# cvigilv/SimSpread.jl

Measured on AMD Instinct MI355X. Metric: predicted edges/sec + achieved HBM GB/s, W*R SpMM, higher is better.
Workload: dtype f32

## Files before the change

### simspread.jl_amd/csrc/assemble.hip

```cpp
#include <cstdlib>
#include <cstring>
#include <hip/hip_runtime.h>
#include <rocprim/rocprim.hpp>

#include "graph.hpp"

namespace ss {

static inline int grid_for(int64_t work, int block, int cap = 256 * 16) {
  int64_t g = ceil_div(work, block);
  if (g < 1) g = 1;
  if (g > cap) g = cap;
  return (int)g;
}

__global__ void scan_tail_kernel(const int* in, int* out, int64_t n) { out[n] = out[n - 1] + in[n - 1]; }

static int exclusive_scan_int(const int* in, int* out, int64_t n) {
  hipStream_t st = ctx().stream;
  if (n == 0) {
    SS_HIP(hipMemsetAsync(out, 0, sizeof(int), st));
    return SS_OK;
  }
  size_t bytes = 0;
// ... 973 lines not shown
    }
  }
}

template <class T>
int csell_build(const DevCsr<T>& in, int KC, int QT, DevCsell<T>& out) {
  hipStream_t st = ctx().stream;
  if (KC < 1 || KC > 32767) return fail(SS_EINVAL, "compact sliced ELL: chunk size out of range");
  const int rowb = QT * (int)sizeof(T);
  if (rowb != 16 && rowb != 32 && rowb != 64 && rowb != 128 && rowb != 256)
    return fail(SS_EINVAL, "compact sliced ELL: tile rows must be 16, 32, 64, 128 or 256 bytes");
  out.ok = false;
  out.rows = in.rows; out.cols = in.cols; out.nnz = in.nnz; out.binary = in.binary;
  out.KC = KC; out.QT = QT;
  out.nchunks = (int)(in.cols > 0 ? ceil_div(in.cols, KC) : 1);
  out.nslices = (int)ceil_div(in.rows, 64);
  const int64_t nblocks = (int64_t)out.nchunks * out.nslices;
  if (nblocks <= 0 || nblocks >= (1LL << 24)) return SS_OK;
  DevBuf<int> steps, pairs, base;
  SS_TRY(out.np.alloc((size_t)(nblocks + 1) * 64));
  SS_TRY(steps.alloc(nblocks + 1));
  SS_TRY(pairs.alloc(nblocks + 1));
  SS_TRY(base.alloc(nblocks + 2));
  SS_HIP(hipMemsetAsync(out.np.p + (size_t)nblocks * 64, 0, 64 * sizeof(unsigned short), st));
  const unsigned grid = (unsigned)(nblocks < (1 << 20) ? nblocks : (1 << 20));
  hipLaunchKernelGGL(csell_count_kernel, dim3(grid), dim3(64), 0, st, in.ptr.p, in.idx.p, in.rows, KC, out.nslices,
                     nblocks, out.np.p, steps.p, pairs.p);
  SS_LAUNCH_CHECK();
  SS_TRY(exclusive_scan_int(pairs.p, base.p, nblocks));
  int total = 0;
  SS_TRY(read_int(base.p + nblocks, &total));
  if (total < 0) return SS_OK;
  out.npairs = total;
  SS_TRY(out.desc.alloc((size_t)(nblocks + 1) * 2));
  hipLaunchKernelGGL(csell_desc_kernel, dim3(grid_for(nblocks + 1, 256)), dim3(256), 0, st, base.p, steps.p, nblocks, out.desc.p);
  SS_LAUNCH_CHECK();
  SS_TRY(out.pidx.alloc((size_t)total + 64));
  SS_HIP(hipMemsetAsync(out.pidx.p + total, 0, 64 * sizeof(unsigned), st));
  if (!in.binary) {
    SS_TRY(out.pval.alloc(2 * ((size_t)total + 64)));
    SS_HIP(hipMemsetAsync(out.pval.p + 2 * (size_t)total, 0, 128 * sizeof(T), st));
  } else {
    out.pval.release();
  }
  DevBuf<int> perm;
  if (rowb < 256) SS_TRY(perm.alloc(in.nnz));
  unsigned short* p16 = reinterpret_cast<unsigned short*>(out.pidx.p);
  T* pv = in.binary ? (T*)nullptr : out.pval.p;
  if (rowb == 16)
    hipLaunchKernelGGL((csell_fill_kernel<T, 16>), dim3(grid), dim3(64), 0, st, in.ptr.p, in.idx.p, in.val.p, in.rows, KC,
                       out.nslices, nblocks, out.desc.p, perm.p, p16, pv);
  else if (rowb == 32)
    hipLaunchKernelGGL((csell_fill_kernel<T, 32>), dim3(grid), dim3(64), 0, st, in.ptr.p, in.idx.p, in.val.p, in.rows, KC,
                       out.nslices, nblocks, out.desc.p, perm.p, p16, pv);
  else if (rowb == 64)
    hipLaunchKernelGGL((csell_fill_kernel<T, 64>), dim3(grid), dim3(64), 0, st, in.ptr.p, in.idx.p, in.val.p, in.rows, KC,
                       out.nslices, nblocks, out.desc.p, perm.p, p16, pv);
  else if (rowb == 128)
    hipLaunchKernelGGL((csell_fill_kernel<T, 128>), dim3(grid), dim3(64), 0, st, in.ptr.p, in.idx.p, in.val.p, in.rows, KC,
                       out.nslices, nblocks, out.desc.p, perm.p, p16, pv);
  else
    hipLaunchKernelGGL((csell_fill_kernel<T, 256>), dim3(grid), dim3(64), 0, st, in.ptr.p, in.idx.p, in.val.p, in.rows, KC,
                       out.nslices, nblocks, out.desc.p, perm.p, p16, pv);
  SS_LAUNCH_CHECK();
  SS_HIP(hipStreamSynchronize(st));
  out.ok = true;
  return SS_OK;
}
template int csell_build<float>(const DevCsr<float>&, int, int, DevCsell<float>&);
template int csell_build<double>(const DevCsr<double>&, int, int, DevCsell<double>&);

template <class T>
__global__ void abs_range_kernel(const T* __restrict__ v, int64_t n, int* __restrict__ mm) {
  int mx = 0, mn = 0x7f7fffff;
  for (int64_t i = (int64_t)blockIdx.x * blockDim.x + threadIdx.x; i < n; i += (int64_t)gridDim.x * blockDim.x) {
    const float a = fabsf((float)v[i]);
    const int b = __float_as_int(a);
    if (a > 0.f) { mx = b > mx ? b : mx; mn = b < mn ? b : mn; }
  }
  atomicMax(&mm[0], mx);
  atomicMin(&mm[1], mn);
}

__global__ void chunk_count_kernel(const int* __restrict__ ptr, const int* __restrict__ idx, int64_t rows, int SC,
                                   int nchunks, int align, int* __restrict__ cnt, unsigned short* __restrict__ len16,
                                   int* __restrict__ toolong) {
  const int64_t total = rows * nchunks;
  for (int64_t i = (int64_t)blockIdx.x * blockDim.x + threadIdx.x; i < total; i += (int64_t)gridDim.x * blockDim.x) {
    const int c = (int)(i / rows);
    const int64_t r = i - (int64_t)c * rows;
    const int lo = ptr[r], hi = ptr[r + 1];
    const int64_t k0 = (int64_t)c * SC, k1 = k0 + SC;
    int a = lo, b = hi;
    while (a < b) { const int m = (a + b) >> 1; if (idx[m] < k0) a = m + 1; else b = m; }
    const int first = a;
    b = hi;
    while (a < b) { const int m = (a + b) >> 1; if (idx[m] < k1) a = m + 1; else b = m; }
    cnt[i] = (a - first + align - 1) / align;
    if (len16) {
      len16[i] = (unsigned short)(a - first);
      if (a - first > 65535) *toolong = 1;
    }
  }
}

constexpr int CHUNK_SCHED_ITERS = 4;
template <class T>
__global__ void chunk_fill_kernel(const int* __restrict__ ptr, const int* __restrict__ idx, const T* __restrict__ val,
                                  int64_t rows, int SC, int nchunks, int align, int sched,
                                  const int* __restrict__ off, unsigned short* __restrict__ oidx, T* __restrict__ oval) {
  const int lane = threadIdx.x & 63;
  const int64_t wave0 = ((int64_t)blockIdx.x * blockDim.x + threadIdx.x) >> 6;
  const int64_t nwaves = ((int64_t)gridDim.x * blockDim.x) >> 6;
  const int64_t total = rows * nchunks;
  for (int64_t i = wave0; i < total; i += nwaves) {
    const int c = (int)(i / rows);
    const int64_t r = i - (int64_t)c * rows;
    const int64_t o = (int64_t)off[i] * align;
    const int npad = (off[i + 1] - off[i]) * align;
    if (npad == 0) continue;
    const int lo = ptr[r], hi = ptr[r + 1];
    const int64_t k0 = (int64_t)c * SC, k1 = k0 + SC;
    int a = lo, b = hi;
    while (a < b) { const int m = (a + b) >> 1; if (idx[m] < k0) a = m + 1; else b = m; }
    const int first = a;
    b = hi;
    while (a < b) { const int m = (a + b) >> 1; if (idx[m] < k1) a = m + 1; else b = m; }
    const int n = a - first;
    if (sched && n > 32 && n <= 64 * CHUNK_SCHED_ITERS) {
      const int G = (n + 31) >> 5;
      const int L = n - 32 * (G - 1);
      int cnt = 0;
      int bank[CHUNK_SCHED_ITERS], col[CHUNK_SCHED_ITERS];
#pragma unroll
      for (int j = 0; j < CHUNK_SCHED_ITERS; ++j) {
        const int x = lane + 64 * j;
        col[j] = x < n ? (int)(idx[first + x] - k0) : -1;
        bank[j] = x < n ? (col[j] & 31) : -1;
      }
      for (int b = 0; b < 32; ++b) {
        int c = 0;
#pragma unroll
        for (int j = 0; j < CHUNK_SCHED_ITERS; ++j) c += __popcll(__ballot(bank[j] == b));
        if (lane == b) cnt = c;
      }
      int base = 0;
      for (int b = 0; b < 31; ++b) {
        const int c = __builtin_amdgcn_readlane(cnt, b);
        if (lane > b) base += c;
      }
      int run = 0;
#pragma unroll
      for (int j = 0; j < CHUNK_SCHED_ITERS; ++j) {
        int p = -1;
        for (int b = 0; b < 32; ++b) {
          const unsigned long long m = __ballot(bank[j] == b);
          const int bb = __builtin_amdgcn_readlane(base, b) + __builtin_amdgcn_readlane(run, b);
          if (bank[j] == b) p = bb + __popcll(m & ((1ull << lane) - 1ull));
          if (lane == b) run += __popcll(m);
        }
        if (p >= 0) {
          int grp, slot;
          if (p < L * G) { grp = p % G; slot = p / G; }
          else { const int q = p - L * G; grp = q % (G - 1); slot = L + q / (G - 1); }
          const int pos = grp * 32 + slot;
          oidx[o + pos] = (unsigned short)col[j];
          oval[o + pos] = val[first + lane + 64 * j];
        }
      }
      for (int x = n + lane; x < npad; x += 64) {
        oidx[o + x] = (unsigned short)SC;
        oval[o + x] = T(0);
      }
      continue;
    }
    for (int x = lane; x < npad; x += 64) {
      oidx[o + x] = x < n ? (unsigned short)(idx[first + x] - k0) : (unsigned short)SC;
      oval[o + x] = x < n ? val[first + x] : T(0);
    }
  }
}

template <class T>
int chunked_build(const DevCsr<T>& in, int SC, int align, DevChunked<T>& out) {
  hipStream_t st = ctx().stream;
  if (SC < 1 || SC > 65535) return fail(SS_EINVAL, "chunk size out of range");
  if (align != 1 && align != 4 && align != 32) return fail(SS_EINVAL, "chunk alignment must be 1, 4 or 32");
  out.rows = in.rows;
  out.cols = in.cols;
  out.nnz = in.nnz;
  out.SC = SC;
  out.align = align;
  out.binary = in.binary;
  out.nchunks = (int)(in.cols > 0 ? ceil_div(in.cols, SC) : 1);
  const int64_t total = in.rows * out.nchunks;
  SS_TRY(out.off.alloc(total + 1));
  if (total == 0) {
    SS_HIP(hipMemsetAsync(out.off.p, 0, sizeof(int), st));
    SS_TRY(out.idx.alloc(64));
    SS_TRY(out.val.alloc(64));
    SS_HIP(hipMemsetAsync(out.idx.p, 0, 64 * sizeof(unsigned short), st));
    SS_HIP(hipMemsetAsync(out.val.p, 0, 64 * sizeof(T), st));
    return SS_OK;
  }
  DevBuf<int> cnt;
  SS_TRY(cnt.alloc(total));
  DevBuf<int> toolong;
  if (align == 32) {
    SS_TRY(out.len.alloc(total));
    SS_TRY(toolong.alloc(1));
    SS_HIP(hipMemsetAsync(toolong.p, 0, sizeof(int), st));
  }
  hipLaunchKernelGGL(chunk_count_kernel, dim3(grid_for(total, 256)), dim3(256), 0, st, in.ptr.p, in.idx.p, in.rows, SC,
                     out.nchunks, align, cnt.p, align == 32 ? out.len.p : (unsigned short*)nullptr,
                     align == 32 ? toolong.p : (int*)nullptr);
  SS_LAUNCH_CHECK();
  if (align == 32) {
    int tl = 0;
    SS_TRY(read_int(toolong.p, &tl));
    out.len_ok = (tl == 0);
  }
  {
    DevBuf<int> mm;
    SS_TRY(mm.alloc(2));
    const int init[2] = {0, 0x7f7fffff};
    SS_HIP(hipMemcpyAsync(mm.p, init, sizeof(init), hipMemcpyHostToDevice, st));
    if (in.nnz > 0) {
      hipLaunchKernelGGL(abs_range_kernel<T>, dim3(grid_for(in.nnz, 256)), dim3(256), 0, st, in.val.p, in.nnz, mm.p);
      SS_LAUNCH_CHECK();
    }
    int got[2];
    SS_HIP(hipMemcpyAsync(got, mm.p, sizeof(got), hipMemcpyDeviceToHost, st));
    SS_HIP(hipStreamSynchronize(st));
    memcpy(&out.vmax, &got[0], 4);
    memcpy(&out.vmin, &got[1], 4);
    if (in.nnz == 0) out.vmax = out.vmin = 0.f;
  }
  SS_TRY(exclusive_scan_int(cnt.p, out.off.p, total));
  int units = 0;
  SS_TRY(read_int(out.off.p + total, &units));
  if (units < 0 || (int64_t)units * align >= (1LL << 31) - 64) return fail(SS_EUNSUPPORTED, "chunked operand too large");
  out.stored = (int64_t)units * align;
  SS_TRY(out.idx.alloc(out.stored + 256));
  SS_TRY(out.val.alloc(out.stored + 256));
  SS_HIP(hipMemsetAsync(out.idx.p + out.stored, 0, 256 * sizeof(unsigned short), st));
  SS_HIP(hipMemsetAsync(out.val.p + out.stored, 0, 256 * sizeof(T), st));
  const int sched = ((align == 1 || align == 32) && !env_off("SS_CHUNK_SCHED")) ? 1 : 0;
  hipLaunchKernelGGL(chunk_fill_kernel<T>, dim3(grid_for(total * 64, 256)), dim3(256), 0, st, in.ptr.p, in.idx.p,
                     in.val.p, in.rows, SC, out.nchunks, align, sched, out.off.p, out.idx.p, out.val.p);
  SS_LAUNCH_CHECK();
  SS_HIP(hipStreamSynchronize(st));
  return SS_OK;
}

template <class T>
__global__ void degree_kernel(const int* __restrict__ pa, const int* __restrict__ pb, int64_t n, int* __restrict__ k,
                              T* __restrict__ inv) {
  for (int64_t i = (int64_t)blockIdx.x * blockDim.x + threadIdx.x; i < n; i += (int64_t)gridDim.x * blockDim.x) {
    int d = pa[i + 1] - pa[i];
    if (pb) d += pb[i + 1] - pb[i];
    k[i] = d;
    inv[i] = d > 0 ? T(1) / T(d) : T(0);
  }
}

template <class T>
int graph_finalize(Graph<T>& g) {
  SS_TRY(csr_transpose(g.Xs, g.XsT));
  SS_TRY(csr_transpose(g.Ys, g.YsT));
  return graph_degrees(g);
}

template <class T>
int graph_degrees(Graph<T>& g) {
  hipStream_t st = ctx().stream;
  g.coef_drop();
  SS_TRY(g.kf.alloc(g.nf));
  SS_TRY(g.ks.alloc(g.ns));
  SS_TRY(g.kt.alloc(g.nt));
  SS_TRY(g.inv_kf.alloc(g.nf));
  SS_TRY(g.inv_ks.alloc(g.ns));
  SS_TRY(g.inv_kt.alloc(g.nt));
  if (g.nf > 0) {
    hipLaunchKernelGGL(degree_kernel<T>, dim3(grid_for(g.nf, 256)), dim3(256), 0, st, g.XsT.ptr.p, (const int*)nullptr,
                       g.nf, g.kf.p, g.inv_kf.p);
    SS_LAUNCH_CHECK();
  }
  if (g.ns > 0) {
    hipLaunchKernelGGL(degree_kernel<T>, dim3(grid_for(g.ns, 256)), dim3(256), 0, st, g.Xs.ptr.p, g.Ys.ptr.p, g.ns,
                       g.ks.p, g.inv_ks.p);
    SS_LAUNCH_CHECK();
  }
  if (g.nt > 0) {
    hipLaunchKernelGGL(degree_kernel<T>, dim3(grid_for(g.nt, 256)), dim3(256), 0, st, g.YsT.ptr.p, (const int*)nullptr,
                       g.nt, g.kt.p, g.inv_kt.p);
    SS_LAUNCH_CHECK();
  }
  SS_HIP(hipStreamSynchronize(st));
  return SS_OK;
}

template <class T>
int graph_finalize_general(Graph<T>& g) {
  hipStream_t st = ctx().stream;
  const int64_t n = g.ns;
  g.coef_drop();
  SS_TRY(g.kf.alloc(n));
  SS_TRY(g.inv_kf.alloc(n));
  SS_TRY(g.ks.alloc(n));
  SS_TRY(g.inv_ks.alloc(n));
  SS_TRY(g.kt.alloc(g.nt));
  SS_TRY(g.inv_kt.alloc(g.nt));
  if (n > 0) {
    hipLaunchKernelGGL(degree_kernel<T>, dim3(grid_for(n, 256)), dim3(256), 0, st, g.XsT.ptr.p, (const int*)nullptr, n,
                       g.kf.p, g.inv_kf.p);
    SS_LAUNCH_CHECK();
    hipLaunchKernelGGL(degree_kernel<T>, dim3(grid_for(n, 256)), dim3(256), 0, st, g.XsT.ptr.p, (const int*)nullptr, n,
                       g.ks.p, g.inv_ks.p);
    SS_LAUNCH_CHECK();
  }
  if (g.nt > 0) {
    hipLaunchKernelGGL(degree_kernel<T>, dim3(grid_for(g.nt, 256)), dim3(256), 0, st, g.YsT.ptr.p, (const int*)nullptr,
                       g.nt, g.kt.p, g.inv_kt.p);
    SS_LAUNCH_CHECK();
  }
  SS_HIP(hipStreamSynchronize(st));
  return SS_OK;
}

template <class T>
int graph_finalize_general_targets(Graph<T>& g) {
  hipStream_t st = ctx().stream;
// ... 27 lines not shown
```

### simspread.jl_amd/csrc/transfer.hip

```cpp
#include <type_traits>

#include "graph.hpp"

namespace ss {

template <class T>
struct ChunkedView {
  const int* off;
  const unsigned short* idx;
  const T* val;
  int64_t rows;
};
template <class T>
static inline ChunkedView<T> view(const DevChunked<T>& m) {
  return ChunkedView<T>{m.off.p, m.idx.p, m.val.p, m.rows};
}

template <class T>
struct TransferArgs {
  int nterms;
  CsrView<T> L[2];
  const T* inv1[2];
  const T* coef[2];
  ChunkedView<T> M[2];
// ... 78 lines not shown
  unsigned b[U];
  T cf[U];
  unsigned short j[U];
  T v[U];
};

template <int U, bool BINM>
__device__ __forceinline__ void subrows_load_buf(SubRows<float, U>& s, int first, int b_l, int n_l, float cf_l,
                                                 __amdgpu_buffer_rsrc_t ridx, __amdgpu_buffer_rsrc_t rval, int lane) {
#pragma unroll
  for (int u = 0; u < U; ++u) {
    const int src = first + u;
    s.b[u] = (unsigned)__builtin_amdgcn_readlane(b_l, src);
    s.n[u] = __builtin_amdgcn_readlane(n_l, src);
    s.cf[u] = BitsOf<float>::bcast(cf_l, src);
    s.j[u] = __builtin_amdgcn_raw_buffer_load_b16(ridx, lane * 2, (int)(s.b[u] * 2u), 0);
    s.v[u] = BINM ? 1.f : __builtin_bit_cast(float, __builtin_amdgcn_raw_buffer_load_b32(rval, lane * 4, (int)(s.b[u] * 4u), 0));
    __builtin_amdgcn_sched_barrier(0);
  }
}

template <class T, int U, bool BINM>
__device__ __forceinline__ void subrows_load(SubRows<T, U>& s, int first, int b_l, int n_l, T cf_l,
                                             const unsigned short* __restrict__ midx, const T* __restrict__ mval,
                                             int lane) {
#pragma unroll
  for (int u = 0; u < U; ++u) {
    const int src = first + u;
    s.b[u] = (unsigned)__builtin_amdgcn_readlane(b_l, src);
    s.n[u] = __builtin_amdgcn_readlane(n_l, src);
    s.cf[u] = BitsOf<T>::bcast(cf_l, src);
    const unsigned short* pi = midx + s.b[u];
    const T* pv = mval + s.b[u];
    s.j[u] = pi[lane];
    s.v[u] = BINM ? T(1) : pv[lane];
    __builtin_amdgcn_sched_barrier(0);
  }
}

template <class T, int U, bool DUAL>
__device__ __forceinline__ void subrows_fold(const SubRows<T, U>& s, T* __restrict__ acc, int astride, int dummy, int lane) {
  if constexpr (DUAL) {
    T* __restrict__ acc1 = acc + astride;
#pragma unroll
    for (int u = 0; u < U; u += 2) {
      const int ja = lane < s.n[u] ? (int)s.j[u] : dummy;
      const int jb = lane < s.n[u + 1] ? (int)s.j[u + 1] : dummy;
      const T ra = acc[ja], rb = acc1[jb];
      acc[ja] = fma(s.cf[u], s.v[u], ra);
      acc1[jb] = fma(s.cf[u + 1], s.v[u + 1], rb);
    }
  } else {
#pragma unroll
    for (int u = 0; u < U; ++u) {
      const int j = lane < s.n[u] ? (int)s.j[u] : dummy;
      acc[j] = fma(s.cf[u], s.v[u], acc[j]);
    }
  }
}

__device__ __forceinline__ int cvt_rpi(float x) {
  int r;
  asm("v_cvt_rpi_i32_f32 %0, %1" : "=v"(r) : "v"(x));
  return r;
}
template <int U>
__device__ __forceinline__ void subrows_fold_fixed(const SubRows<float, U>& s, unsigned* __restrict__ acc, int lane) {
#pragma unroll
  for (int u = 0; u < U; ++u) {
    const float v = lane < s.n[u] ? s.v[u] : 0.f;
    atomicAdd(&acc[s.j[u]], (unsigned)cvt_rpi(s.cf[u] * v));
  }
}

template <class T, int U, bool DUAL, bool FIX>
__device__ __forceinline__ void subrows_fold_any(const SubRows<T, U>& s, T* acc, int astride, int dummy, int lane) {
  if constexpr (FIX) subrows_fold_fixed<U>(s, reinterpret_cast<unsigned*>(acc), lane);
  else subrows_fold<T, U, DUAL>(s, acc, astride, dummy, lane);
}

template <class T, int AHEAD>
struct Tails {
  static constexpr int TAIL_AHEAD = AHEAD;
  int nt;
  int cb, cn;
  T ccf;
  unsigned short tj[TAIL_AHEAD];
  T tv[TAIL_AHEAD];
};

template <class T, int TAIL_AHEAD, class LD>
__device__ __forceinline__ void tails_fetch(Tails<T, TAIL_AHEAD>& t, int r0, int lane, LD&& ld) {
#pragma unroll
  for (int i = 0; i < TAIL_AHEAD; ++i) {
    if (4 * (r0 + i) >= t.nt) break;
    const unsigned b = (unsigned)__builtin_amdgcn_ds_bpermute((4 * (r0 + i) + (lane >> 4)) * 4, t.cb);
    ld(b + 64u + (unsigned)(lane & 15), t.tj[i], t.tv[i]);
    __builtin_amdgcn_sched_barrier(0);
  }
}

template <class T, int TAIL_AHEAD, class LD>
__device__ __forceinline__ void tails_begin(Tails<T, TAIL_AHEAD>& t, int b_l, int n_l, T cf_l, int lane, LD&& ld) {
  const unsigned long long longs = __ballot(n_l > 64);
  t.nt = __builtin_popcountll(longs);
  if (t.nt == 0) return;
  const int k = (int)__builtin_amdgcn_mbcnt_hi((unsigned)(longs >> 32), __builtin_amdgcn_mbcnt_lo((unsigned)longs, 0u));
  const int to4 = (n_l > 64 ? k : t.nt + lane - k) * 4;
  t.cb = __builtin_amdgcn_ds_permute(to4, b_l);
  t.cn = __builtin_amdgcn_ds_permute(to4, n_l);
  t.ccf = BitsOf<T>::push(to4, cf_l);
  tails_fetch(t, 0, lane, ld);
}

template <class T, bool BINM, bool FIX, int TAIL_AHEAD, class LD>
__device__ __forceinline__ void tails_finish(Tails<T, TAIL_AHEAD>& t, int b_l, int n_l, T cf_l, T* __restrict__ acc, int dummy,
                                             const unsigned short* __restrict__ midx, const T* __restrict__ mval, int lane,
                                             LD&& ld) {
  if (t.nt == 0) return;
  for (int r0 = 0; 4 * r0 < t.nt; r0 += TAIL_AHEAD) {
    if (r0 > 0) tails_fetch(t, r0, lane, ld);
#pragma unroll
    for (int i = 0; i < TAIL_AHEAD; ++i) {
      if (4 * (r0 + i) >= t.nt) break;
      const int from4 = (4 * (r0 + i) + (lane >> 4)) * 4;
      const int tn = __builtin_amdgcn_ds_bpermute(from4, t.cn) - 64;
      const T tcf = BitsOf<T>::pull(from4, t.ccf);
      const bool live = (lane & 15) < tn;
      if constexpr (FIX) {
        atomicAdd(reinterpret_cast<unsigned*>(acc) + (live ? (int)t.tj[i] : dummy),
                  (unsigned)cvt_rpi(live ? (float)(tcf * t.tv[i]) : 0.f));
      } else {
#pragma unroll
        for (int g = 0; g < 4; ++g) {
          const int j = (live && (lane >> 4) == g) ? (int)t.tj[i] : dummy;
          acc[j] = fma(tcf, t.tv[i], acc[j]);
        }
      }
    }
  }
  unsigned long long m = __ballot(n_l > 80);
  while (m != 0ull) {
    const int src = __builtin_ctzll(m);
    m &= m - 1ull;
    const int n = __builtin_amdgcn_readlane(n_l, src);
    const unsigned b = (unsigned)__builtin_amdgcn_readlane(b_l, src);
    const T cf = BitsOf<T>::bcast(cf_l, src);
    for (int x = 80 + lane; x < n; x += 64) {
      const int j = midx[b + x];
      const T v = BINM ? T(1) : mval[b + x];
      if constexpr (FIX) atomicAdd(reinterpret_cast<unsigned*>(acc) + j, (unsigned)cvt_rpi((float)(cf * v)));
      else acc[j] = fma(cf, v, acc[j]);
    }
  }
}

struct FixedScale {
  float scale, unscale;
};
template <class F>
__device__ __forceinline__ FixedScale fixed_scale(int lb, int le, int lane, float xmax, F&& abs_coef) {
  float sabs = 0.f;
  for (int q = lb + lane; q < le; q += 64) sabs += abs_coef(q);
#pragma unroll
  for (int o = 32; o > 0; o >>= 1) sabs += __shfl_xor(sabs, o);
  int e = 0;
  (void)frexpf(sabs * xmax, &e);
  if (!(sabs * xmax > 0.f)) e = 0;
  e = e < -90 ? -90 : (e > 120 ? 120 : e);
  return FixedScale{ldexpf(1.f, 30 - e), ldexpf(1.f, e - 30)};
}

template <class T, bool LOO, int U, bool BINM, bool DUAL, bool FIX = false, bool BUF = false, bool COEF = false>
__global__ void __launch_bounds__(TRANSFER_THREADS) transfer_kernel(TransferArgs<T> p) {
  static_assert(64 % (2 * U) == 0, "U must divide 32");
  static_assert(!COEF || (!DUAL && !FIX && !BUF), "coefficient tables serve the default family only");
  extern __shared__ __align__(16) unsigned char smem_raw[];
  T* acc = reinterpret_cast<T*>(smem_raw);
  const int astride = p.SC + 64;
  constexpr int NCOPY = DUAL ? 2 : 1;
  unsigned* bits = reinterpret_cast<unsigned*>(acc + NCOPY * astride);
  const int lane = threadIdx.x;
  int c;
  int64_t r;
  if (p.nchunks > 8 && p.nchunks % 8 == 0 && !chunks_in_turn(p)) {
    const int64_t nrows = (int64_t)gridDim.x / p.nchunks, per = nrows * 8;
    const int64_t grp = blockIdx.x / per, rem = blockIdx.x - grp * per;
    r = rem >> 3;
    c = (int)(grp * 8 + (rem & 7));
  } else {
    c = blockIdx.x % p.nchunks;
    r = blockIdx.x / p.nchunks;
  }
  const int64_t gr = p.row_ids ? (int64_t)p.row_ids[p.row_begin + r] : p.row_begin + r;
  const int64_t j0 = (int64_t)c * p.SC;
  const int jn = (int)((p.nj - j0 < p.SC) ? (p.nj - j0) : p.SC);
  const int dummy = p.SC + lane;

  for (int j = lane; j < NCOPY * astride; j += 64) acc[j] = T(0);
  if (LOO)
    for (int j = lane; j < (p.SC + 31) / 32; j += 64) bits[j] = 0u;
  __syncthreads();

  float fix_unscale = 1.f;
  for (int t = 0; t < p.nterms; ++t) {
    const CsrView<T> L = p.L[t];
    const ChunkedView<T> M = p.M[t];
    const int* __restrict__ off = M.off + (int64_t)c * M.rows;
    const unsigned short* __restrict__ midx = M.idx;
    const T* __restrict__ mval = M.val;
    const int lb = L.ptr[gr], le = L.ptr[gr + 1];
    float scale = 1.f;
    if constexpr (FIX) {
      float sabs = 0.f;
      for (int q = lb + lane; q < le; q += 64) sabs += fabsf((float)(L.val[q] * p.inv1[t][L.idx[q]]));
#pragma unroll
      for (int o = 32; o > 0; o >>= 1) sabs += __shfl_xor(sabs, o);
      int e = 0;
      (void)frexpf(sabs * p.xmax, &e);
      if (!(sabs * p.xmax > 0.f)) e = 0;
      e = e < -90 ? -90 : (e > 120 ? 120 : e);
      scale = ldexpf(1.f, 30 - e);
      fix_unscale = ldexpf(1.f, e - 30);
    }
    for (int g0 = lb; g0 < le; g0 += 64) {
      const int q = g0 + lane;
      int b_l = 0, n_l = 0;
      T cf_l = T(0);
      if constexpr (COEF) {
        if (q < le) {
          const int a = L.idx[q];
          cf_l = p.coef[t][q];
          const int o0 = off[a], o1 = off[a + 1];
          b_l = o0;
          n_l = cf_l != T(0) ? o1 - o0 : 0;
        }
      } else if (q < le) {
        const int a = L.idx[q];
        const T lv = L.val[q];
        if (LOO) {
          const int d = p.kf[a] - 1;
          cf_l = (a != (int)gr && d > 0) ? lv * (T(1) / T(d)) : T(0);
        } else {
          cf_l = lv * p.inv1[t][a];
          if constexpr (FIX) cf_l = (T)((float)cf_l * scale);
        }
        if (cf_l != T(0)) { b_l = off[a]; n_l = off[a + 1] - b_l; }
      }
      const int cnt = __builtin_amdgcn_readfirstlane((le - g0 < 64) ? (le - g0) : 64);
      SubRows<T, U> A, B;
      auto load = [&](SubRows<T, U>& sr, int first) __attribute__((always_inline)) {
        if constexpr (BUF) {
          const __amdgpu_buffer_rsrc_t ridx = __builtin_amdgcn_make_buffer_rsrc((void*)midx, 0, -1, 0x00020000);
          const __amdgpu_buffer_rsrc_t rval = __builtin_amdgcn_make_buffer_rsrc((void*)mval, 0, -1, 0x00020000);
          subrows_load_buf<U, BINM>(sr, first, b_l, n_l, cf_l, ridx, rval, lane);
        } else {
          subrows_load<T, U, BINM>(sr, first, b_l, n_l, cf_l, midx, mval, lane);
        }
      };
      auto tail_ld = [&](unsigned e, unsigned short& j, T& v) __attribute__((always_inline)) {
        if constexpr (BUF) {
          const __amdgpu_buffer_rsrc_t ridx = __builtin_amdgcn_make_buffer_rsrc((void*)midx, 0, -1, 0x00020000);
          const __amdgpu_buffer_rsrc_t rval = __builtin_amdgcn_make_buffer_rsrc((void*)mval, 0, -1, 0x00020000);
          j = __builtin_amdgcn_raw_buffer_load_b16(ridx, (int)(e * 2u), 0, 0);
          v = BINM ? 1.f : __builtin_bit_cast(float, __builtin_amdgcn_raw_buffer_load_b32(rval, (int)(e * 4u), 0, 0));
        } else {
          j = midx[e];
          v = BINM ? T(1) : mval[e];
        }
      };
      Tails<T, (BINM ? 4 : 2)> tails;
      tails_begin(tails, b_l, n_l, cf_l, lane, tail_ld);
      load(A, 0);
      for (int u0 = 0; u0 < cnt; u0 += 2 * U) {
        if (u0 + U < cnt) load(B, u0 + U);
        subrows_fold_any<T, U, DUAL, FIX>(A, acc, astride, dummy, lane);
        if (u0 + U < cnt) {
          if (u0 + 2 * U < cnt) load(A, u0 + 2 * U);
          subrows_fold_any<T, U, DUAL, FIX>(B, acc, astride, dummy, lane);
        }
      }
      tails_finish<T, BINM, FIX>(tails, b_l, n_l, cf_l, acc, dummy, midx, mval, lane, tail_ld);
    }
  }
  if (LOO) {
    const ChunkedView<T> M = p.M[0];
    const int* off = M.off + (int64_t)c * M.rows;
    for (int x = off[gr] + lane; x < off[gr + 1]; x += 64) {
      const int j = M.idx[x];
      atomicOr(&bits[j >> 5], 1u << (j & 31));
    }
  }
  __syncthreads();

  T* orow = p.out + r * p.ld + j0;
  for (int j = lane; j < jn; j += 64) {
    T z;
    T sum = DUAL ? acc[j] + acc[astride + j] : acc[j];
    if constexpr (FIX) sum = (T)((float)reinterpret_cast<const int*>(acc)[j] * fix_unscale);
    if (LOO) {
      const int d = p.ks[j0 + j] - (int)((bits[j >> 5] >> (j & 31)) & 1u);
      z = (d > 0 && (j0 + j) != gr) ? sum * (T(1) / T(d)) : T(0);
    } else {
      z = sum * p.inv2[j0 + j];
      if (p.accumulate) z += orow[j];
    }
    orow[j] = z;
  }
}

constexpr int TRANSFER_U = 8;

static bool transfer_dual() { return env_int("SS_TRANSFER_DUAL", 0) != 0; }

static int transfer_u() {
  const int u = (int)env_int("SS_TRANSFER_U", TRANSFER_U);
  return (u == 4 || u == 16) ? u : 8;
}

template <class T>
__global__ void transfer_coef_kernel(const int* __restrict__ ptr, const int* __restrict__ idx, const T* __restrict__ val,
                                     const T* __restrict__ inv1, int64_t row_begin, int64_t nrows, T* __restrict__ coef) {
  const int lo = ptr[row_begin], hi = ptr[row_begin + nrows];
  for (int64_t e = (int64_t)lo + (int64_t)blockIdx.x * blockDim.x + threadIdx.x; e < hi; e += (int64_t)gridDim.x * blockDim.x)
    coef[e] = val[e] * inv1[idx[e]];
}

enum { TB_PLAIN, TB_QFLAT, TB_WIDE, TB_WIDE2 };
constexpr int WIDE_META = 64 * 12;
constexpr int WIDE_LIST = 64;
constexpr int W2_TBL = 64 * 12;
template <int KIND, class T>
struct BlockLayout {
  static constexpr bool EXACT = KIND != TB_PLAIN;
  static constexpr int shared_bytes = KIND == TB_WIDE ? 64 : 0;
  __host__ __device__ static int64_t offs_bytes(int64_t mrows) { return (((mrows + 1) * 4 + 15) / 16) * 16; }
  __host__ __device__ static int64_t lens_bytes(int64_t mrows) { return EXACT ? ((mrows * 2 + 15) / 16) * 16 : 0; }
  __host__ __device__ static int acc_elems(int SC) { return SC + 64; }
  __host__ __device__ static int acc_bytes(int SC) {
    return KIND == TB_WIDE || KIND == TB_WIDE2 ? (((SC + 4) * 4 + 15) / 16) * 16 : acc_elems(SC) * (int)sizeof(T);
  }
  __host__ __device__ static int per_wave(int SC) {
    return acc_bytes(SC) + (KIND == TB_WIDE ? WIDE_META + WIDE_LIST : KIND == TB_WIDE2 ? 2 * W2_TBL + 4 * 64 : 0);
  }
  __device__ static unsigned char* wave_base(unsigned char* smem, int offs_b, int lens_b, int wave, int SC) {
    return smem + offs_b + lens_b + shared_bytes + (size_t)wave * (size_t)per_wave(SC);
  }
};

struct BlockWave {
  int lane, c, jn, lb, le;
  int64_t r, gr, j0;
};

template <bool EXACT, class T, class A>
__device__ __forceinline__ bool block_prologue(BlockWave& w, const TransferArgs<T>& p, int64_t nrows, int wave, int* offs,
                                               unsigned short* lens, const unsigned short* glen, A* acc, int nacc) {
  const int nw = blockDim.x >> 6;
  w.lane = threadIdx.x & 63;
  w.c = blockIdx.x % p.nchunks;
  w.r = (int64_t)(blockIdx.x / p.nchunks) * nw + wave;
  const ChunkedView<T> M = p.M[0];
  {
    const int* __restrict__ off = M.off + (int64_t)w.c * M.rows;
    for (int64_t i = threadIdx.x; i <= M.rows; i += blockDim.x) offs[i] = off[i];
    if constexpr (EXACT) {
      const unsigned short* __restrict__ gl = glen + (int64_t)w.c * M.rows;
      for (int64_t i = threadIdx.x; i < M.rows; i += blockDim.x) lens[i] = gl[i];
    }
  }
  for (int j = w.lane; j < nacc; j += 64) acc[j] = A(0);
  __syncthreads();
  return w.r < nrows;
}
template <class T>
__device__ __forceinline__ void block_row(BlockWave& w, const TransferArgs<T>& p) {
  w.gr = p.row_begin + w.r;
  w.j0 = (int64_t)w.c * p.SC;
  w.jn = (int)((p.nj - w.j0 < p.SC) ? (p.nj - w.j0) : p.SC);
  const int* lptr = p.L[0].ptr;
  w.lb = __builtin_amdgcn_readfirstlane(lptr[w.gr]);
  w.le = __builtin_amdgcn_readfirstlane(lptr[w.gr + 1]);
}

template <class T>
__device__ __forceinline__ void fixed_store(const TransferArgs<T>& p, int64_t r, int64_t j0, int jn, int lane, const void* acc,
                                            float unscale) {
  T* orow = p.out + r * p.ld + j0;
  const int* iacc = reinterpret_cast<const int*>(acc);
  for (int j = lane; j < jn; j += 64) orow[j] = (T)((float)iacc[j] * unscale) * p.inv2[j0 + j];
}

typedef float f4 __attribute__((ext_vector_type(4)));
typedef unsigned u2 __attribute__((ext_vector_type(2)));

template <bool BINM>
__device__ __forceinline__ void quad_fetch(const u2* midx4, const f4* mval4, int quad, float cfv, int rem, u2& oj, f4& ov,
                                           float& ocf) {
  ocf = cfv;
  oj = midx4[quad];
  if constexpr (BINM) ov = f4{rem > 0 ? 1.f : 0.f, rem > 1 ? 1.f : 0.f, rem > 2 ? 1.f : 0.f, rem > 3 ? 1.f : 0.f};
  else ov = mval4[quad];
}
__device__ __forceinline__ void quad_fold(unsigned* acc, u2 j, f4 v, float cf) {
  atomicAdd(acc + (j.x & 0xffffu), (unsigned)cvt_rpi(cf * v.x));
  atomicAdd(acc + (j.x >> 16), (unsigned)cvt_rpi(cf * v.y));
  atomicAdd(acc + (j.y & 0xffffu), (unsigned)cvt_rpi(cf * v.z));
  atomicAdd(acc + (j.y >> 16), (unsigned)cvt_rpi(cf * v.w));
}

__device__ __forceinline__ void raw_load(const int* lidx, const float* coef, int lb, int le, int lane, int g, int& a, float& cf) {
  const int q = lb + g * 64 + lane;
  a = 0;
  cf = 0.f;
  if (q < le) { a = lidx[q]; cf = coef[q]; }
}

template <class T, int U, bool BINM, bool FIX>
__global__ void __launch_bounds__(1024) transfer_block_kernel(TransferArgs<T> p, const T* __restrict__ coef, int64_t nrows,
                                                              int align, int offs_bytes, float xmax) {
  using Lay = BlockLayout<TB_PLAIN, T>;
  extern __shared__ __align__(16) unsigned char smem_raw[];
  int* offs = reinterpret_cast<int*>(smem_raw);
  const int wave = threadIdx.x >> 6;
  const int astride = p.SC + 64;
  T* acc = reinterpret_cast<T*>(smem_raw + offs_bytes) + (size_t)wave * Lay::acc_elems(p.SC);
  BlockWave w;
  if (!block_prologue<false>(w, p, nrows, wave, offs, nullptr, nullptr, acc, astride)) return;
  w.gr = p.row_begin + w.r;
  w.j0 = (int64_t)w.c * p.SC;
  w.jn = (int)((p.nj - w.j0 < p.SC) ? (p.nj - w.j0) : p.SC);
  const int lane = w.lane, lb = p.L[0].ptr[w.gr], le = p.L[0].ptr[w.gr + 1];
  const int dummy = p.SC + lane;
  const CsrView<T> L = p.L[0];
  const unsigned short* __restrict__ midx = p.M[0].idx;
  const T* __restrict__ mval = p.M[0].val;
  float scale = 1.f, unscale = 1.f;
  if constexpr (FIX) {
    const FixedScale fs = fixed_scale(lb, le, lane, xmax, [&](int q) __attribute__((always_inline)) { return fabsf((float)coef[q]); });
    scale = fs.scale;
    unscale = fs.unscale;
  }
  for (int g0 = lb; g0 < le; g0 += 64) {
    const int q = g0 + lane;
    int b_l = 0, n_l = 0;
    T cf_l = T(0);
    if (q < le) {
      const int a = L.idx[q];
      cf_l = coef[q];
      if constexpr (FIX) cf_l = (T)((float)cf_l * scale);
      if (cf_l != T(0)) {
        const int o0 = offs[a], o1 = offs[a + 1];
        b_l = o0 * align;
        n_l = (o1 - o0) * align;
      }
    }
    const int cnt = __builtin_amdgcn_readfirstlane((le - g0 < 64) ? (le - g0) : 64);
    SubRows<T, U> A, B;
    auto load = [&](SubRows<T, U>& sr, int first) __attribute__((always_inline)) {
      subrows_load<T, U, BINM>(sr, first, b_l, n_l, cf_l, midx, mval, lane);
    };
    auto tail_ld = [&](unsigned e, unsigned short& j, T& v) __attribute__((always_inline)) {
      j = midx[e];
      v = BINM ? T(1) : mval[e];
    };
    Tails<T, (BINM ? 4 : 2)> tails;
    tails_begin(tails, b_l, n_l, cf_l, lane, tail_ld);
    load(A, 0);
    for (int u0 = 0; u0 < cnt; u0 += 2 * U) {
      if (u0 + U < cnt) load(B, u0 + U);
      subrows_fold_any<T, U, false, FIX>(A, acc, astride, dummy, lane);
      if (u0 + U < cnt) {
        if (u0 + 2 * U < cnt) load(A, u0 + 2 * U);
        subrows_fold_any<T, U, false, FIX>(B, acc, astride, dummy, lane);
      }
    }
    tails_finish<T, BINM, FIX>(tails, b_l, n_l, cf_l, acc, dummy, midx, mval, lane, tail_ld);
  }
  if constexpr (FIX) {
    fixed_store(p, w.r, w.j0, w.jn, lane, acc, unscale);
  } else {
    T* orow = p.out + w.r * p.ld + w.j0;
    for (int j = lane; j < w.jn; j += 64) orow[j] = acc[j] * p.inv2[w.j0 + j];
  }
}

template <class T, int D, bool BINM>
__global__ void __launch_bounds__(1024) transfer_qflat_kernel(TransferArgs<T> p, const T* __restrict__ coef, int64_t nrows,
                                                             int align, int offs_bytes, int lens_bytes, float xmax,
                                                             const unsigned short* __restrict__ glen) {
  static_assert(std::is_same<T, float>::value, "fixed-point sums: fp32 graphs only");
  extern __shared__ __align__(16) unsigned char smem_raw[];
  int* offs = reinterpret_cast<int*>(smem_raw);
  unsigned short* lens = reinterpret_cast<unsigned short*>(smem_raw + offs_bytes);
  const int lane = threadIdx.x & 63;
  const int wave = __builtin_amdgcn_readfirstlane(threadIdx.x >> 6);
  const int astride = p.SC + 64;
  unsigned* acc = reinterpret_cast<unsigned*>(BlockLayout<TB_QFLAT, T>::wave_base(smem_raw, offs_bytes, lens_bytes, wave, p.SC));
  BlockWave w;
  if (!block_prologue<true>(w, p, nrows, wave, offs, lens, glen, acc, astride)) return;
  block_row(w, p);
  const ChunkedView<T> M = p.M[0];
  const CsrView<T> L = p.L[0];
  const int64_t r = w.r, j0 = w.j0;
  const int jn = w.jn, lb = w.lb, le = w.le;
  const unsigned short* __restrict__ midx = M.idx;
  const T* __restrict__ mval = M.val;
  float scale, unscale;
  {
    float sabs = 0.f;
    for (int q = lb + lane; q < le; q += 64) sabs += fabsf(coef[q]);
#pragma unroll
    for (int o = 32; o > 0; o >>= 1) sabs += __shfl_xor(sabs, o);
    int e = 0;
    (void)frexpf(sabs * xmax, &e);
    if (!(sabs * xmax > 0.f)) e = 0;
    e = e < -90 ? -90 : (e > 120 ? 120 : e);
    scale = ldexpf(1.f, 30 - e);
    unscale = ldexpf(1.f, e - 30);
  }
  const int ngroups = (le - lb + 63) >> 6;
  auto raw_load = [&](int g, int& a, float& cf) __attribute__((always_inline)) {
    const int q = lb + g * 64 + lane;
    a = 0;
    cf = 0.f;
    if (q < le) { a = L.idx[q]; cf = coef[q]; }
  };
  auto meta = [&](int a, float cf, int& b_l, int& n_l, float& cf_l) __attribute__((always_inline)) {
    cf_l = cf * scale;
    b_l = 0;
    n_l = 0;
    if (cf_l != 0.f) {
      b_l = (offs[a] * align) >> 2;
      n_l = ((int)lens[a] + 3) >> 2;
    }
  };
  int Pc = 0, dc = 0, ra, bn, nn;
  float cc = 0.f, cn, rc;
  int total = 0, nst = 0, t = 0, gcur = -1;
  raw_load(0, ra, rc); meta(ra, rc, bn, nn, cn);
  raw_load(1, ra, rc);
  bool done = false;
  auto switch_group = [&]() __attribute__((always_inline)) {
    ++gcur;
    int incl = nn;
#pragma unroll
    for (int o = 1; o < 64; o <<= 1) {
      const int up = __shfl_up(incl, o);
      if (lane >= o) incl += up;
    }
// ... 559 lines not shown
```

Measured before the change: 52.90 billion.

## Class-partition chunk tails so tail atomics avoid bank conflicts across quarter-waves

Chunk assembly now reorders long chunk rows so that the 16-entry tail after the first 64 entries holds columns whose low two bits match the row's class (row mod 4). The SpMM tail processing then groups long rows by class into quarter-wave slots, so each 16-lane group updates accumulator entries in a distinct LDS bank class. This lets the four-way serialized per-group update collapse into a single update. It also rewrites the bank-scheduling fill for up to 64 entries and adds padding and overflow paths, at the cost of a more complex build and extra padding storage.

```diff
diff --git a/simspread.jl_amd/csrc/assemble.hip b/simspread.jl_amd/csrc/assemble.hip
--- a/simspread.jl_amd/csrc/assemble.hip
+++ b/simspread.jl_amd/csrc/assemble.hip
@@ -1079,9 +1079,20 @@
   atomicMin(&mm[1], mn);
 }
 
+struct ChunkTail {
+  int real;
+  int len;
+  int stored;
+};
+__device__ __forceinline__ ChunkTail chunk_tail(int n, int m) {
+  const int t = n - 64 < 16 ? n - 64 : 16;
+  if (m >= t) return ChunkTail{t, t, n};
+  return ChunkTail{m, 16, n + 16 - m};
+}
+
 __global__ void chunk_count_kernel(const int* __restrict__ ptr, const int* __restrict__ idx, int64_t rows, int SC,
-                                   int nchunks, int align, int* __restrict__ cnt, unsigned short* __restrict__ len16,
-                                   int* __restrict__ toolong) {
+                                   int nchunks, int align, int cls_tails, int* __restrict__ cnt,
+                                   unsigned short* __restrict__ len16, int* __restrict__ toolong) {
   const int64_t total = rows * nchunks;
   for (int64_t i = (int64_t)blockIdx.x * blockDim.x + threadIdx.x; i < total; i += (int64_t)gridDim.x * blockDim.x) {
     const int c = (int)(i / rows);
@@ -1093,23 +1104,47 @@
     const int first = a;
     b = hi;
     while (a < b) { const int m = (a + b) >> 1; if (idx[m] < k1) a = m + 1; else b = m; }
-    cnt[i] = (a - first + align - 1) / align;
+    int n = a - first;
+    if (cls_tails && n > 64) {
+      const int cls = (int)(r & 3);
+      int m = 0;
+      for (int x = first; x < a; ++x) m += (int)(((idx[x] - k0) & 3) == cls);
+      n = chunk_tail(n, m).stored;
+    }
+    cnt[i] = (n + align - 1) / align;
     if (len16) {
-      len16[i] = (unsigned short)(a - first);
-      if (a - first > 65535) *toolong = 1;
-    }
-  }
-}
-
-constexpr int CHUNK_SCHED_ITERS = 4;
-template <class T>
-__global__ void chunk_fill_kernel(const int* __restrict__ ptr, const int* __restrict__ idx, const T* __restrict__ val,
-                                  int64_t rows, int SC, int nchunks, int align, int sched,
-                                  const int* __restrict__ off, unsigned short* __restrict__ oidx, T* __restrict__ oval) {
+      len16[i] = (unsigned short)n;
+      if (n > 65535) *toolong = 1;
+    }
+  }
+}
+
+__device__ __forceinline__ int chunk_sched_pos(int n, int col, int lane) {
+  const int bank = col < 0 ? -1 : (col & 31);
+  int p = 0, base = 0;
+  for (int b = 0; b < 32; ++b) {
+    const unsigned long long m = __ballot(bank == b);
+    if (bank == b) p = base + __popcll(m & ((1ull << lane) - 1ull));
+    base += __popcll(m);
+  }
+  const int L = n - 32;
+  return p < 2 * L ? (p & 1) * 32 + (p >> 1) : L + (p - 2 * L);
+}
+
+template <class T>
+__global__ void __launch_bounds__(256) chunk_fill_kernel(const int* __restrict__ ptr, const int* __restrict__ idx,
+                                                         const T* __restrict__ val, int64_t rows, int SC, int nchunks,
+                                                         int align, int sched, int cls_tails,
+                                                         const int* __restrict__ off, unsigned short* __restrict__ oidx,
+                                                         T* __restrict__ oval) {
+  __shared__ int hcol[4][64];
+  __shared__ T hval[4][64];
   const int lane = threadIdx.x & 63;
+  const int wv = (threadIdx.x >> 6) & 3;
   const int64_t wave0 = ((int64_t)blockIdx.x * blockDim.x + threadIdx.x) >> 6;
   const int64_t nwaves = ((int64_t)gridDim.x * blockDim.x) >> 6;
   const int64_t total = rows * nchunks;
+  const unsigned long long below = (1ull << lane) - 1ull;
   for (int64_t i = wave0; i < total; i += nwaves) {
     const int c = (int)(i / rows);
     const int64_t r = i - (int64_t)c * rows;
@@ -1124,46 +1159,63 @@
     b = hi;
     while (a < b) { const int m = (a + b) >> 1; if (idx[m] < k1) a = m + 1; else b = m; }
     const int n = a - first;
-    if (sched && n > 32 && n <= 64 * CHUNK_SCHED_ITERS) {
-      const int G = (n + 31) >> 5;
-      const int L = n - 32 * (G - 1);
-      int cnt = 0;
-      int bank[CHUNK_SCHED_ITERS], col[CHUNK_SCHED_ITERS];
-#pragma unroll
-      for (int j = 0; j < CHUNK_SCHED_ITERS; ++j) {
-        const int x = lane + 64 * j;
-        col[j] = x < n ? (int)(idx[first + x] - k0) : -1;
-        bank[j] = x < n ? (col[j] & 31) : -1;
+    if (cls_tails && n > 64) {
+      const int cls = (int)(r & 3);
+      int m = 0;
+      for (int x0 = 0; x0 < n; x0 += 64) {
+        const int x = x0 + lane;
+        m += __popcll(__ballot(x < n && ((idx[first + x] - k0) & 3) == cls));
       }
-      for (int b = 0; b < 32; ++b) {
-        int c = 0;
-#pragma unroll
-        for (int j = 0; j < CHUNK_SCHED_ITERS; ++j) c += __popcll(__ballot(bank[j] == b));
-        if (lane == b) cnt = c;
+      const ChunkTail tl = chunk_tail(n, m);
+      int seen_c = 0, seen_o = 0;
+      for (int x0 = 0; x0 < n; x0 += 64) {
+        const int x = x0 + lane;
+        const bool valid = x < n;
+        const int col = valid ? (int)(idx[first + x] - k0) : 0;
+        const T v = valid ? val[first + x] : T(0);
+        const unsigned long long mc = __ballot(valid && (col & 3) == cls);
+        const int rc = seen_c + __popcll(mc & below);
+        const bool in_tail = valid && (col & 3) == cls && rc < tl.real;
+        const unsigned long long mo = __ballot(valid && !in_tail);
+        const int ro = seen_o + __popcll(mo & below);
+        if (in_tail) {
+          oidx[o + 64 + rc] = (unsigned short)col;
+          oval[o + 64 + rc] = v;
+        } else if (valid) {
+          if (ro < 64) {
+            hcol[wv][ro] = col;
+            hval[wv][ro] = v;
+          } else {
+            oidx[o + 16 + ro] = (unsigned short)col;
+            oval[o + 16 + ro] = v;
+          }
+        }
+        seen_c += __popcll(mc);
+        seen_o += __popcll(mo);
       }
-      int base = 0;
-      for (int b = 0; b < 31; ++b) {
-        const int c = __builtin_amdgcn_readlane(cnt, b);
-        if (lane > b) base += c;
+      for (int x = tl.real + lane; x < tl.len; x += 64) {
+        oidx[o + 64 + x] = (unsigned short)SC;
+        oval[o + 64 + x] = T(0);
       }
-      int run = 0;
-#pragma unroll
-      for (int j = 0; j < CHUNK_SCHED_ITERS; ++j) {
-        int p = -1;
-        for (int b = 0; b < 32; ++b) {
-          const unsigned long long m = __ballot(bank[j] == b);
-          const int bb = __builtin_amdgcn_readlane(base, b) + __builtin_amdgcn_readlane(run, b);
-          if (bank[j] == b) p = bb + __popcll(m & ((1ull << lane) - 1ull));
-          if (lane == b) run += __popcll(m);
-        }
-        if (p >= 0) {
-          int grp, slot;
-          if (p < L * G) { grp = p % G; slot = p / G; }
-          else { const int q = p - L * G; grp = q % (G - 1); slot = L + q / (G - 1); }
-          const int pos = grp * 32 + slot;
-          oidx[o + pos] = (unsigned short)col[j];
-          oval[o + pos] = val[first + lane + 64 * j];
-        }
+      __builtin_amdgcn_wave_barrier();
+      const int hc = hcol[wv][lane];
+      const T hv = hval[wv][lane];
+      __builtin_amdgcn_wave_barrier();
+      const int pos = sched ? chunk_sched_pos(64, hc, lane) : lane;
+      oidx[o + pos] = (unsigned short)hc;
+      oval[o + pos] = hv;
+      for (int x = tl.stored + lane; x < npad; x += 64) {
+        oidx[o + x] = (unsigned short)SC;
+        oval[o + x] = T(0);
+      }
+      continue;
+    }
+    if (sched && n > 32 && n <= 64) {
+      const int col = lane < n ? (int)(idx[first + lane] - k0) : -1;
+      const int pos = chunk_sched_pos(n, col, lane);
+      if (lane < n) {
+        oidx[o + pos] = (unsigned short)col;
+        oval[o + pos] = val[first + lane];
       }
       for (int x = n + lane; x < npad; x += 64) {
         oidx[o + x] = (unsigned short)SC;
@@ -1202,6 +1254,7 @@
   }
   DevBuf<int> cnt;
   SS_TRY(cnt.alloc(total));
+  const int cls_tails = (align == 1 || align == 32) ? 1 : 0;
   DevBuf<int> toolong;
   if (align == 32) {
     SS_TRY(out.len.alloc(total));
@@ -1209,7 +1262,7 @@
     SS_HIP(hipMemsetAsync(toolong.p, 0, sizeof(int), st));
   }
   hipLaunchKernelGGL(chunk_count_kernel, dim3(grid_for(total, 256)), dim3(256), 0, st, in.ptr.p, in.idx.p, in.rows, SC,
-                     out.nchunks, align, cnt.p, align == 32 ? out.len.p : (unsigned short*)nullptr,
+                     out.nchunks, align, cls_tails, cnt.p, align == 32 ? out.len.p : (unsigned short*)nullptr,
                      align == 32 ? toolong.p : (int*)nullptr);
   SS_LAUNCH_CHECK();
   if (align == 32) {
@@ -1242,9 +1295,9 @@
   SS_TRY(out.val.alloc(out.stored + 256));
   SS_HIP(hipMemsetAsync(out.idx.p + out.stored, 0, 256 * sizeof(unsigned short), st));
   SS_HIP(hipMemsetAsync(out.val.p + out.stored, 0, 256 * sizeof(T), st));
-  const int sched = ((align == 1 || align == 32) && !env_off("SS_CHUNK_SCHED")) ? 1 : 0;
+  const int sched = (cls_tails && !env_off("SS_CHUNK_SCHED")) ? 1 : 0;
   hipLaunchKernelGGL(chunk_fill_kernel<T>, dim3(grid_for(total * 64, 256)), dim3(256), 0, st, in.ptr.p, in.idx.p,
-                     in.val.p, in.rows, SC, out.nchunks, align, sched, out.off.p, out.idx.p, out.val.p);
+                     in.val.p, in.rows, SC, out.nchunks, align, sched, cls_tails, out.off.p, out.idx.p, out.val.p);
   SS_LAUNCH_CHECK();
   SS_HIP(hipStreamSynchronize(st));
   return SS_OK;
diff --git a/simspread.jl_amd/csrc/transfer.hip b/simspread.jl_amd/csrc/transfer.hip
--- a/simspread.jl_amd/csrc/transfer.hip
+++ b/simspread.jl_amd/csrc/transfer.hip
@@ -184,7 +184,8 @@
 template <class T, int AHEAD>
 struct Tails {
   static constexpr int TAIL_AHEAD = AHEAD;
-  int nt;
+  int nr;
+  unsigned long long ovf;
   int cb, cn;
   T ccf;
   unsigned short tj[TAIL_AHEAD];
@@ -195,7 +196,7 @@
 __device__ __forceinline__ void tails_fetch(Tails<T, TAIL_AHEAD>& t, int r0, int lane, LD&& ld) {
 #pragma unroll
   for (int i = 0; i < TAIL_AHEAD; ++i) {
-    if (4 * (r0 + i) >= t.nt) break;
+    if (r0 + i >= t.nr) break;
     const unsigned b = (unsigned)__builtin_amdgcn_ds_bpermute((4 * (r0 + i) + (lane >> 4)) * 4, t.cb);
     ld(b + 64u + (unsigned)(lane & 15), t.tj[i], t.tv[i]);
     __builtin_amdgcn_sched_barrier(0);
@@ -203,14 +204,32 @@
 }
 
 template <class T, int TAIL_AHEAD, class LD>
-__device__ __forceinline__ void tails_begin(Tails<T, TAIL_AHEAD>& t, int b_l, int n_l, T cf_l, int lane, LD&& ld) {
-  const unsigned long long longs = __ballot(n_l > 64);
-  t.nt = __builtin_popcountll(longs);
-  if (t.nt == 0) return;
-  const int k = (int)__builtin_amdgcn_mbcnt_hi((unsigned)(longs >> 32), __builtin_amdgcn_mbcnt_lo((unsigned)longs, 0u));
-  const int to4 = (n_l > 64 ? k : t.nt + lane - k) * 4;
-  t.cb = __builtin_amdgcn_ds_permute(to4, b_l);
-  t.cn = __builtin_amdgcn_ds_permute(to4, n_l);
+__device__ __forceinline__ void tails_begin(Tails<T, TAIL_AHEAD>& t, int a_l, int b_l, int n_l, T cf_l, int lane, LD&& ld) {
+  const bool lng = n_l > 64;
+  const unsigned long long longs = __ballot(lng);
+  t.nr = 0;
+  if (longs == 0ull) return;
+  const int cls = a_l & 3;
+  int k = 0, rounds = 0, fewest = 16, spare = 0, taken = 0;
+#pragma unroll
+  for (int c = 0; c < 4; ++c) {
+    const unsigned long long mc = __ballot(lng && cls == c);
+    const int kc = (int)__builtin_amdgcn_mbcnt_hi((unsigned)(mc >> 32), __builtin_amdgcn_mbcnt_lo((unsigned)mc, 0u));
+    int cc = __builtin_popcountll(mc);
+    cc = cc < 16 ? cc : 16;
+    k = cls == c ? kc : k;
+    rounds = cc > rounds ? cc : rounds;
+    if (cc < fewest) { fewest = cc; spare = 4 * cc + c; }
+    taken = (lane & 3) == c ? cc : taken;
+  }
+  const bool placed = lng && k < 16;
+  t.nr = rounds;
+  t.ovf = __ballot(lng && k >= 16);
+  const int to4 = (placed ? 4 * k + cls : spare) * 4;
+  const bool mine = (lane >> 2) < taken;
+  const int pb = __builtin_amdgcn_ds_permute(to4, b_l), pn = __builtin_amdgcn_ds_permute(to4, n_l);
+  t.cb = mine ? pb : 0;
+  t.cn = mine ? pn : 0;
   t.ccf = BitsOf<T>::push(to4, cf_l);
   tails_fetch(t, 0, lane, ld);
 }
@@ -219,12 +238,12 @@
 __device__ __forceinline__ void tails_finish(Tails<T, TAIL_AHEAD>& t, int b_l, int n_l, T cf_l, T* __restrict__ acc, int dummy,
                                              const unsigned short* __restrict__ midx, const T* __restrict__ mval, int lane,
                                              LD&& ld) {
-  if (t.nt == 0) return;
-  for (int r0 = 0; 4 * r0 < t.nt; r0 += TAIL_AHEAD) {
+  if (t.nr == 0) return;
+  for (int r0 = 0; r0 < t.nr; r0 += TAIL_AHEAD) {
     if (r0 > 0) tails_fetch(t, r0, lane, ld);
 #pragma unroll
     for (int i = 0; i < TAIL_AHEAD; ++i) {
-      if (4 * (r0 + i) >= t.nt) break;
+      if (r0 + i >= t.nr) break;
       const int from4 = (4 * (r0 + i) + (lane >> 4)) * 4;
       const int tn = __builtin_amdgcn_ds_bpermute(from4, t.cn) - 64;
       const T tcf = BitsOf<T>::pull(from4, t.ccf);
@@ -233,22 +252,19 @@
         atomicAdd(reinterpret_cast<unsigned*>(acc) + (live ? (int)t.tj[i] : dummy),
                   (unsigned)cvt_rpi(live ? (float)(tcf * t.tv[i]) : 0.f));
       } else {
-#pragma unroll
-        for (int g = 0; g < 4; ++g) {
-          const int j = (live && (lane >> 4) == g) ? (int)t.tj[i] : dummy;
-          acc[j] = fma(tcf, t.tv[i], acc[j]);
-        }
+        const int j = live ? (int)t.tj[i] : dummy;
+        acc[j] = fma(tcf, t.tv[i], acc[j]);
       }
     }
   }
-  unsigned long long m = __ballot(n_l > 80);
+  unsigned long long m = __ballot(n_l > 80) | t.ovf;
   while (m != 0ull) {
     const int src = __builtin_ctzll(m);
     m &= m - 1ull;
     const int n = __builtin_amdgcn_readlane(n_l, src);
     const unsigned b = (unsigned)__builtin_amdgcn_readlane(b_l, src);
     const T cf = BitsOf<T>::bcast(cf_l, src);
-    for (int x = 80 + lane; x < n; x += 64) {
+    for (int x = (((t.ovf >> src) & 1ull) ? 64 : 80) + lane; x < n; x += 64) {
       const int j = midx[b + x];
       const T v = BINM ? T(1) : mval[b + x];
       if constexpr (FIX) atomicAdd(reinterpret_cast<unsigned*>(acc) + j, (unsigned)cvt_rpi((float)(cf * v)));
@@ -327,18 +343,18 @@
     }
     for (int g0 = lb; g0 < le; g0 += 64) {
       const int q = g0 + lane;
-      int b_l = 0, n_l = 0;
+      int a_l = 0, b_l = 0, n_l = 0;
       T cf_l = T(0);
       if constexpr (COEF) {
         if (q < le) {
-          const int a = L.idx[q];
+          const int a = a_l = L.idx[q];
           cf_l = p.coef[t][q];
           const int o0 = off[a], o1 = off[a + 1];
           b_l = o0;
           n_l = cf_l != T(0) ? o1 - o0 : 0;
         }
       } else if (q < le) {
-        const int a = L.idx[q];
+        const int a = a_l = L.idx[q];
         const T lv = L.val[q];
         if (LOO) {
           const int d = p.kf[a] - 1;
@@ -371,8 +387,8 @@
           v = BINM ? T(1) : mval[e];
         }
       };
-      Tails<T, (BINM ? 4 : 2)> tails;
-      tails_begin(tails, b_l, n_l, cf_l, lane, tail_ld);
+      Tails<T, (BINM ? 4 : (DUAL || FIX || BUF) ? 2 : 3)> tails;
+      tails_begin(tails, a_l, b_l, n_l, cf_l, lane, tail_ld);
       load(A, 0);
       for (int u0 = 0; u0 < cnt; u0 += 2 * U) {
         if (u0 + U < cnt) load(B, u0 + U);
@@ -390,7 +406,7 @@
     const int* off = M.off + (int64_t)c * M.rows;
     for (int x = off[gr] + lane; x < off[gr + 1]; x += 64) {
       const int j = M.idx[x];
-      atomicOr(&bits[j >> 5], 1u << (j & 31));
+      if (j < p.SC) atomicOr(&bits[j >> 5], 1u << (j & 31));
     }
   }
   __syncthreads();
@@ -545,10 +561,10 @@
   }
   for (int g0 = lb; g0 < le; g0 += 64) {
     const int q = g0 + lane;
-    int b_l = 0, n_l = 0;
+    int a_l = 0, b_l = 0, n_l = 0;
     T cf_l = T(0);
     if (q < le) {
-      const int a = L.idx[q];
+      const int a = a_l = L.idx[q];
       cf_l = coef[q];
       if constexpr (FIX) cf_l = (T)((float)cf_l * scale);
       if (cf_l != T(0)) {
@@ -567,7 +583,7 @@
       v = BINM ? T(1) : mval[e];
     };
     Tails<T, (BINM ? 4 : 2)> tails;
-    tails_begin(tails, b_l, n_l, cf_l, lane, tail_ld);
+    tails_begin(tails, a_l, b_l, n_l, cf_l, lane, tail_ld);
     load(A, 0);
     for (int u0 = 0; u0 < cnt; u0 += 2 * U) {
       if (u0 + U < cnt) load(B, u0 + U);
```

After: 53.49 billion (median of 6 runs). 1.01x the previous value.
